# CVMI-Lab/DODA

Measured on AMD Instinct MI355X. Metric: active-voxels/sec fwd+bwd SparseConv U-Net, ScanNet 2cm, higher is better.
Workload: dtype bf16; 1 GPU; cfgs/scannet SparseConv U-Net training step (voxel pooling + fwd + CE + bwd + SGD), 2 cm voxels, 4 scenes/GPU x ~150000 active voxels, random-init weights; global_batch=4, voxels_per_gpu=601279, points_per_gpu=781042, parallelism=dp1, n_classes=20, grad_sync=deferred multi-layer wgrad + bucketed all-reduce, collectives=none (single process), prefetch_gate=off, grad_exchange=no process group

## Files before the change

doda_amd/csrc/spconv_tile.hip:

```cpp
#include "common.hpp"
#include "tilebook.hpp"
#include "spconv_common.hpp"

#ifdef DODA_TILE_STAMPS
__device__ unsigned long long doda_tile_stamp_buf[768 * 8 * 8];
extern "C" int doda_debug_tile_stamps(void *host_out, size_t bytes) {
    return (int)hipMemcpyFromSymbol(host_out, HIP_SYMBOL(doda_tile_stamp_buf), bytes);
}
#define TILE_STAMP(k)                                                                                      \
    do {                                                                                                   \
        if (tid0 == 0 && stamp_it < 8) doda_tile_stamp_buf[(blockIdx.x * 8 + stamp_it) * 8 + (k)] = wall_clock64(); \
    } while (0)
#else
#define TILE_STAMP(k) do { } while (0)
#endif

namespace {

template <bool OUT32> struct EpiPre { u32x4 res[4], bnx[4]; };
template <> struct EpiPre<false> { u32x2 res[4], bnx[4]; };

template <int S, bool OUT32, bool STATS, bool ALWAYS = false>
__device__ __forceinline__ void epi_prefetch(EpiPre<OUT32> &pre, int row0, int i, int g, int nb0, int nc, int n_out,
                                             unsigned y_bytes, const void *__restrict__ res, const EpiArgs &ep) {
    constexpr unsigned OSZ = OUT32 ? 4u : 2u;
    const unsigned col = (unsigned)(nb0 * 16 + 4 * g);
    const unsigned rl = ep.res_ld ? ep.res_ld : (unsigned)nc, bl = ep.bnx_ld ? ep.bnx_ld : (unsigned)nc;
    const unsigned dense_bytes = (unsigned)n_out * (unsigned)nc * OSZ;
    const unsigned r_bytes = ep.res_ld ? ((unsigned)(n_out - 1) * rl + (unsigned)nc) * OSZ : (ep.y_ld ? dense_bytes : y_bytes);
    const unsigned b_bytes = ep.bnx_ld ? ((unsigned)(n_out - 1) * bl + (unsigned)nc) * OSZ : (ep.y_ld ? dense_bytes : y_bytes);
    const __amdgpu_buffer_rsrc_t rs_r = __builtin_amdgcn_make_buffer_rsrc((void *)res, 0, r_bytes, 0x00020000);
    const __amdgpu_buffer_rsrc_t rs_b = __builtin_amdgcn_make_buffer_rsrc((void *)ep.bn_x, 0, b_bytes, 0x00020000);
#pragma unroll
    for (int s = 0; s < S; ++s) {
        const unsigned t = (unsigned)(row0 + s * 16 + i);
        const bool in_range = t < (unsigned)n_out && col < (unsigned)nc;
        const unsigned voff = in_range ? (t * rl + col) * OSZ : OOB;
        const unsigned voff_b = in_range ? (t * bl + col) * OSZ : OOB;
        if constexpr (ALWAYS) {
            const unsigned vr = res ? voff : OOB, vb = ep.bn_x ? voff_b : OOB;
            if constexpr (OUT32) pre.res[s] = __builtin_amdgcn_raw_buffer_load_b128(rs_r, vr, 0, 0);
            else pre.res[s] = __builtin_amdgcn_raw_buffer_load_b64(rs_r, vr, 0, 0);
            if constexpr (STATS) {
                if constexpr (OUT32) pre.bnx[s] = __builtin_amdgcn_raw_buffer_load_b128(rs_b, vb, 0, 0);
                else pre.bnx[s] = __builtin_amdgcn_raw_buffer_load_b64(rs_b, vb, 0, 0);
            }
            continue;
        }
        if (res) {
            if constexpr (OUT32) pre.res[s] = __builtin_amdgcn_raw_buffer_load_b128(rs_r, voff, 0, 0);
            else pre.res[s] = __builtin_amdgcn_raw_buffer_load_b64(rs_r, voff, 0, 0);
        }
        if (STATS && ep.bn_x) {
            if constexpr (OUT32) pre.bnx[s] = __builtin_amdgcn_raw_buffer_load_b128(rs_b, voff_b, 0, 0);
            else pre.bnx[s] = __builtin_amdgcn_raw_buffer_load_b64(rs_b, voff_b, 0, 0);
        }
    }
}

__device__ __forceinline__ f32x4 epi_unpack(const u32x4 &v) { return __builtin_bit_cast(f32x4, v); }
__device__ __forceinline__ f32x4 epi_unpack(const u32x2 &v) {
    return (f32x4){__uint_as_float(v[0] << 16), __uint_as_float(v[0] & 0xffff0000u),
                   __uint_as_float(v[1] << 16), __uint_as_float(v[1] & 0xffff0000u)};
}

template <int S, bool OUT32, bool STATS, bool BNLDS = false, int B = 0, int NBA = 1>
__device__ __forceinline__ void tile_epilogue(f32x4 (&acc)[S][NBA], const EpiPre<OUT32> &pre, int row0, int i, int g,
                                              int nb0, int nc, int n_out, __amdgpu_buffer_rsrc_t rs_y,
                                              const void *__restrict__ res, const EpiArgs &ep, f32x4 (&lst)[2],
                                              const f32x4 (*bnv_lds)[4] = nullptr) {
    constexpr unsigned OSZ = OUT32 ? 4u : 2u;
    const unsigned col = (unsigned)(nb0 * 16 + 4 * g);
    f32x4 st1 = {0.f, 0.f, 0.f, 0.f}, st2 = {0.f, 0.f, 0.f, 0.f};
    f32x4 mu = {0.f, 0.f, 0.f, 0.f}, is = mu, ga = mu, be = mu;
    if constexpr (STATS) {
        if (BNLDS && ep.bn_x) {
            mu = bnv_lds[0][g];
            is = bnv_lds[1][g];
            ga = bnv_lds[2][g];
            be = bnv_lds[3][g];
        } else if (!BNLDS && ep.bn_x) {
            const unsigned cc = col < (unsigned)nc ? col : 0u;
            mu = *reinterpret_cast<const f32x4 *>(ep.bn_mean + cc);
            is = *reinterpret_cast<const f32x4 *>(ep.bn_invstd + cc);
            if (ep.bn_relu) {
                ga = *reinterpret_cast<const f32x4 *>(ep.bn_gamma + cc);
                be = *reinterpret_cast<const f32x4 *>(ep.bn_beta + cc);
            }
        }
    }
    const unsigned yl = ep.y_ld ? ep.y_ld : (unsigned)nc;
#pragma unroll
    for (int s = 0; s < S; ++s) {
        const unsigned t = (unsigned)(row0 + s * 16 + i);
        const unsigned voff = (t < (unsigned)n_out && col < (unsigned)nc) ? (t * yl + col) * OSZ : OOB;
        f32x4 a = acc[s][B];
        if (res) a += epi_unpack(pre.res[s]);
        u32x2 packed_out = {0u, 0u};
        if constexpr (!OUT32) {
            packed_out[0] = (unsigned)f2bf(a[0]) | ((unsigned)f2bf(a[1]) << 16);
            packed_out[1] = (unsigned)f2bf(a[2]) | ((unsigned)f2bf(a[3]) << 16);
        }
        if constexpr (STATS) {
            f32x4 v = a;
            if constexpr (!OUT32) v = epi_unpack(packed_out);
            if (ep.bn_x) {
                const f32x4 xr = epi_unpack(pre.bnx[s]);
                const f32x4 xh = (xr - mu) * is;
                if (ep.bn_relu) {
                    const f32x4 yv = xh * ga + be;
#pragma unroll
                    for (int q = 0; q < 4; ++q) v[q] = yv[q] > 0.f ? v[q] : 0.f;
                }
                st1 += v;
                st2 += v * xh;
            } else {
                st1 += v;
                st2 += v * v;
            }
        }
        if constexpr (OUT32)
            __builtin_amdgcn_raw_buffer_store_b128(__builtin_bit_cast(u32x4, a), rs_y, voff, 0, 0);
        else
            __builtin_amdgcn_raw_buffer_store_b64(packed_out, rs_y, voff, 0, 0);
    }
    if constexpr (STATS) {
        lst[0] += st1;
        lst[1] += st2;
    }
}

__device__ __forceinline__ void stats_flush(f32x4 (&lst)[2], int i, int g, int wid, int nb0, int nc, const EpiArgs &ep, long long part) {
    __shared__ f32x4 sred[4][2][4];
    f32x4 st1 = lst[0], st2 = lst[1];
#pragma unroll
    for (int q = 0; q < 4; ++q) { st1[q] = row_sum16(st1[q]); st2[q] = row_sum16(st2[q]); }
    if (i == 15) { sred[wid][0][g] = st1; sred[wid][1][g] = st2; }
    doda_sync();
    const int col = nb0 * 16 + 4 * g;
    if (wid == 0 && i == 15 && col < nc) {
        const f32x4 a1 = (sred[0][0][g] + sred[1][0][g]) + (sred[2][0][g] + sred[3][0][g]);
        const f32x4 a2 = (sred[0][1][g] + sred[1][1][g]) + (sred[2][1][g] + sred[3][1][g]);
        stats_emit(ep, part, nc, col, a1, a2);
    }
    doda_sync();
}

template <int MODE, bool OUT32, bool STATS, int MAXNB, bool DUAL = false>
__global__ __launch_bounds__(256, MODE == 0 ? 3 : 2) void conv_tile(const void *__restrict__ x, unsigned x_bytes,
                                                 const void *__restrict__ wp, unsigned wp_bytes, int nc, int NB,
                                                 const int32_t *__restrict__ tbl, int ld, int n_out,
                                                 const TileBookView tb, void *__restrict__ y, unsigned y_bytes,
                                                 const void *__restrict__ res, const EpiArgs ep) {
    constexpr bool WIDE = MODE != 0;
    static_assert(MODE != 2 || OUT32, "fp32 features have fp32 outputs");
    static_assert(!DUAL || (MODE == 1 && (MAXNB == 2 || MAXNB == 4 || !STATS)), "two channel blocks per pass: bf16, 64-byte rows");
    static_assert(MAXNB != 4 || DUAL, "statistics of four channel blocks: two dual passes");
    constexpr int NBA = DUAL ? 2 : 1;
    constexpr int S = 4, NU = WIDE ? TB_K : (TB_K + 1) / 2;
    constexpr int RB = WIDE ? 64 : 32;
    constexpr int PPR = RB / 16;
    constexpr int CAP = WIDE ? TB_CAP64 : TB_LMAX;
    constexpr int NLJ = PPR;
    constexpr int NRL = 4 * NLJ;
    constexpr int NLP = TB_LIDX_BYTES / 16;
    constexpr int NLI = (NLP + 255) / 256;
    __shared__ __attribute__((aligned(16))) unsigned char rows_s[(CAP + 1) * RB];
    __shared__ __attribute__((aligned(16))) unsigned lidx_s[TB_T * TB_LW];
    static_assert(MAXNB == 1 || MAXNB == 2 || MAXNB == 4, "statistics of one, two or (dual passes) four channel blocks");
    f32x4 lst[STATS ? MAXNB : 1][2];
#pragma unroll
    for (int b = 0; b < (STATS ? MAXNB : 1); ++b) lst[b][0] = lst[b][1] = (f32x4){0.f, 0.f, 0.f, 0.f};

    const int tid0 = threadIdx.x, wid = __builtin_amdgcn_readfirstlane(tid0 >> 6);
    const __amdgpu_buffer_rsrc_t rs_x = __builtin_amdgcn_make_buffer_rsrc((void *)x, 0, x_bytes, 0x00020000);
    const __amdgpu_buffer_rsrc_t rs_w = __builtin_amdgcn_make_buffer_rsrc((void *)wp, 0, wp_bytes, 0x00020000);
    const __amdgpu_buffer_rsrc_t rs_y = __builtin_amdgcn_make_buffer_rsrc((void *)y, 0, y_bytes, 0x00020000);
    const __amdgpu_buffer_rsrc_t rs_t = __builtin_amdgcn_make_buffer_rsrc((void *)tbl, 0, (unsigned)TB_K * (unsigned)ld * 4u, 0x00020000);

    const int L = gridDim.x >> 3, xcd = blockIdx.x & 7, slot = blockIdx.x >> 3;
    const int qn = tb.nt >> 3, rn = tb.nt & 7;
    const int lo = xcd < rn ? xcd * (qn + 1) : rn * (qn + 1) + (xcd - rn) * qn;
    const int cnt = qn + (xcd < rn ? 1 : 0);

    auto entry_of = [&](int j, int k, int tid) { return j * (256 / PPR) + tid / PPR + 256 * k; };
    auto load_list = [&](int tile, int tid, unsigned (&rid)[NRL]) {
        const u32x4 *ul4 = reinterpret_cast<const u32x4 *>(tb.ulist + (size_t)tile * TB_UMAX);
#pragma unroll
        for (int j = 0; j < NLJ; ++j) {
            const u32x4 v = ul4[j * (256 / PPR) + tid / PPR];
#pragma unroll
            for (int k = 0; k < 4; ++k) rid[4 * j + k] = v[k];
        }
    };
    unsigned rid[NRL];
    int U = 0;
    if (slot < cnt) {
        load_list(lo + slot, tid0, rid);
        U = tb.ucount[lo + slot];
    }
#ifdef DODA_TILE_STAMPS
    int stamp_it = -1;
#endif
    for (int tt = slot; tt < cnt; tt += L) {
        const int tile = lo + tt, t0 = tile * TB_T;
#ifdef DODA_TILE_STAMPS
        ++stamp_it;
#endif
        TILE_STAMP(0);
        int tid = tid0;
        asm volatile("" : "+v"(tid));
        const int lane = tid & 63, i = lane & 15, g = lane >> 4;
        const bool staged = U <= CAP;
        const int row0 = t0 + wid * 64;
        const unsigned half = (unsigned)(WIDE ? g : (g & 1)) * 16u;
        unsigned lane_w = WIDE ? (unsigned)lane * 16u
                               : (unsigned)(g >> 1) * (unsigned)NB * 512u + (unsigned)((g & 1) * 16 + i) * 16u;
        auto loadw = [&](int u, int b = 0) {
            return __builtin_amdgcn_raw_buffer_load_b128(rs_w, (unsigned)u * (unsigned)NB * 1024u + lane_w + (unsigned)b * (WIDE ? 1024u : 512u), 0, 0);
        };
        EpiPre<OUT32> pre;
        epi_prefetch<S, OUT32, STATS>(pre, row0, i, g, 0, nc, n_out, y_bytes, res, ep);

        if (staged) {
            u32x4 rr[NRL];
#pragma unroll
            for (int k = 0; k < NRL; ++k)
                rr[k] = __builtin_amdgcn_raw_buffer_load_b128(rs_x, rid[k] * (unsigned)RB + (unsigned)(tid & (PPR - 1)) * 16u, 0, 0);
            u32x4 li4[NLI];
            const u32x4 *li = reinterpret_cast<const u32x4 *>(tb.lidx + (size_t)tile * (TB_T * TB_LW));
#pragma unroll
            for (int k = 0; k < NLI; ++k) {
                const int e = k * 256 + tid;
                li4[k] = li[e < NLP ? e : 0];
            }
            if (tt + L < cnt) {
                load_list(tile + L, tid, rid);
                U = tb.ucount[tile + L];
            }
#pragma unroll
            for (int k = 0; k < NLI; ++k) {
                const int e = k * 256 + tid;
                if (e < NLP) reinterpret_cast<u32x4 *>(lidx_s)[e] = li4[k];
            }
            if (tid < PPR) reinterpret_cast<u32x4 *>(rows_s)[tid] = (u32x4){0u, 0u, 0u, 0u};
#pragma unroll
            for (int k = 0; k < NRL; ++k) {
                const int e = entry_of(k >> 2, k & 3, tid);
                if (e < CAP) reinterpret_cast<u32x4 *>(rows_s)[PPR + e * PPR + (tid & (PPR - 1))] = rr[k];
            }
        } else {
            static_assert((CAP + 1) * RB >= TB_K * TB_T * 4, "the table slice fits the row buffer");
            int te[TB_K];
            unsigned ldv = (unsigned)ld;
            asm volatile("" : "+s"(ldv));
#pragma unroll
            for (int o = 0; o < TB_K; ++o) {
                const unsigned voff = (unsigned)(t0 + tid) < (unsigned)n_out ? ((unsigned)o * ldv + (unsigned)(t0 + tid)) * 4u : OOB;
                te[o] = (int)__builtin_amdgcn_raw_buffer_load_b32(rs_t, voff, 0, 0);
            }
            if (tt + L < cnt) {
                load_list(tile + L, tid, rid);
                U = tb.ucount[tile + L];
            }
            int *tab_s = reinterpret_cast<int *>(rows_s);
#pragma unroll
            for (int o = 0; o < TB_K; ++o) tab_s[o * TB_T + tid] = (unsigned)(t0 + tid) < (unsigned)n_out ? te[o] : -1;
        }
        TILE_STAMP(1);
        doda_sync();
        TILE_STAMP(2);

        for (int nb0 = 0; nb0 < NB; nb0 += NBA) {
            if (nb0 > 0) {
                lane_w += (WIDE ? 1024u : 512u) * (unsigned)NBA;
                epi_prefetch<S, OUT32, STATS>(pre, row0, i, g, nb0, nc, n_out, y_bytes, res, ep);
            }

            f32x4 acc[S][NBA];
#pragma unroll
            for (int s = 0; s < S; ++s)
#pragma unroll
                for (int b = 0; b < NBA; ++b) acc[s][b] = (f32x4){0.f, 0.f, 0.f, 0.f};
            if (staged) {
                const unsigned *my = lidx_s + wid * 64 + tb_lsigma(i) * 4 + ((!WIDE && (g >> 1)) ? 5 * TB_T : 0);
                auto loadp = [&](int plane) { return *reinterpret_cast<const u32x4 *>(my + plane * TB_T); };
                constexpr int NSTR = WIDE ? 2 : 1;
                u32x4 lw[NSTR][2];
                auto word_of = [&](int u) -> const u32x4 & { return WIDE ? lw[u & 1][((u >> 1) / 3) & 1] : lw[0][(u / 3) & 1]; };
                auto fetch = [&](int u, u32x4 (&xa)[S]) {
                    const unsigned sh = WIDE ? 10u * (unsigned)((u >> 1) % 3) : 10u * (unsigned)(u % 3);
                    const u32x4 &l = word_of(u);
#pragma unroll
                    for (int s = 0; s < S; ++s)
                        xa[s] = *reinterpret_cast<const u32x4 *>(rows_s + ((__builtin_amdgcn_ubfe(l[s], sh, 10u) * (unsigned)RB) | half));
                };
                auto next_word = [&](int u) {
                    if constexpr (WIDE) {
                        const int p = u & 1, k = (u >> 1) / 3;
                        if ((u >> 1) % 3 == 0 && 2 * (3 * (k + 1)) + p < TB_K) lw[p][(k + 1) & 1] = loadp(5 * p + k + 1);
                    } else {
                        const int k = u / 3;
                        if (u % 3 == 0 && 3 * (k + 1) < NU) lw[0][(k + 1) & 1] = loadp(k + 1);
                    }
                };
                u32x4 xa[2][S], wr[4][NBA];
#pragma unroll
                for (int u = 0; u < 3; ++u)
#pragma unroll
                    for (int b = 0; b < NBA; ++b) wr[u][b] = loadw(u, b);
                lw[0][0] = loadp(0);
                if constexpr (WIDE) lw[1][0] = loadp(5);
                fetch(0, xa[0]);
#pragma unroll
                for (int u = 0; u < NU; ++u) {
                    if (u + 1 < NU) fetch(u + 1, xa[(u + 1) & 1]);
                    next_word(u);
                    if (u + 3 < NU) {
#pragma unroll
                        for (int b = 0; b < NBA; ++b) wr[(u + 3) & 3][b] = loadw(u + 3, b);
                    }
                    __builtin_amdgcn_sched_barrier(0);
#pragma unroll
                    for (int s = 0; s < S; ++s) {
#pragma unroll
                        for (int b = 0; b < NBA; ++b) {
                            if constexpr (MODE == 2) mma_f32_k16<false>(acc[s][b], wr[u & 3][b], xa[u & 1][s]);
                            else mma_bf16_k32(acc[s][b], wr[u & 3][b], xa[u & 1][s]);
                        }
                    }
                    __builtin_amdgcn_sched_barrier(0);
                }
            } else {
                const int *tab_s = reinterpret_cast<const int *>(rows_s) + wid * 64 + i;
                auto ldi = [&](int u, int (&d)[S]) {
                    const int osel = WIDE ? u : 2 * u + (g >> 1);
#pragma unroll
                    for (int s = 0; s < S; ++s) d[s] = osel < TB_K ? tab_s[osel * TB_T + s * 16] : -1;
                };
                auto ldx = [&](const int (&d)[S], u32x4 (&xr)[S]) {
#pragma unroll
                    for (int s = 0; s < S; ++s)
                        xr[s] = __builtin_amdgcn_raw_buffer_load_b128(rs_x, d[s] >= 0 ? (unsigned)d[s] * (unsigned)RB + half : OOB, 0, 0);
                };
                int ix[3][S];
                u32x4 xo[2][S];
                ldi(0, ix[0]);
                ldi(1, ix[1]);
                ldx(ix[0], xo[0]);
#pragma unroll
                for (int u = 0; u < NU; ++u) {
                    if (u + 2 < NU) ldi(u + 2, ix[(u + 2) % 3]);
                    if (u + 1 < NU) ldx(ix[(u + 1) % 3], xo[(u + 1) & 1]);
                    u32x4 wu[NBA];
#pragma unroll
                    for (int b = 0; b < NBA; ++b) wu[b] = loadw(u, b);
#pragma unroll
                    for (int s = 0; s < S; ++s) {
#pragma unroll
                        for (int b = 0; b < NBA; ++b) {
                            if constexpr (MODE == 2) mma_f32_k16<false>(acc[s][b], wu[b], xo[u & 1][s]);
                            else mma_bf16_k32(acc[s][b], wu[b], xo[u & 1][s]);
                        }
                    }
                }
            }
            TILE_STAMP(3);
            if constexpr (DUAL) {
                EpiPre<OUT32> pre1;
                epi_prefetch<S, OUT32, STATS>(pre1, row0, i, g, nb0 + 1, nc, n_out, y_bytes, res, ep);
                if (MAXNB == 4 && nb0 == 2) {
                    tile_epilogue<S, OUT32, STATS, false, 0, NBA>(acc, pre, row0, i, g, nb0, nc, n_out, rs_y, res, ep, lst[STATS && MAXNB == 4 ? 2 : 0]);
                    tile_epilogue<S, OUT32, STATS, false, 1, NBA>(acc, pre1, row0, i, g, nb0 + 1, nc, n_out, rs_y, res, ep, lst[STATS && MAXNB == 4 ? 3 : 0]);
                } else {
                    tile_epilogue<S, OUT32, STATS, false, 0, NBA>(acc, pre, row0, i, g, nb0, nc, n_out, rs_y, res, ep, lst[0]);
                    tile_epilogue<S, OUT32, STATS, false, 1, NBA>(acc, pre1, row0, i, g, nb0 + 1, nc, n_out, rs_y, res, ep, lst[STATS && MAXNB > 1 ? 1 : 0]);
                }
            } else {
                if (nb0 == 0) tile_epilogue<S, OUT32, STATS>(acc, pre, row0, i, g, nb0, nc, n_out, rs_y, res, ep, lst[0]);
                else tile_epilogue<S, OUT32, STATS>(acc, pre, row0, i, g, nb0, nc, n_out, rs_y, res, ep, lst[STATS ? MAXNB - 1 : 0]);
            }
        }
        TILE_STAMP(4);
        doda_sync();
        TILE_STAMP(5);
    }
    if constexpr (STATS) {
        const int lane = tid0 & 63, i = lane & 15, g = lane >> 4;
        stats_flush(lst[0], i, g, wid, 0, nc, ep, (long long)blockIdx.x);
#pragma unroll
        for (int b = 1; b < MAXNB; ++b)
            if (b < NB) stats_flush(lst[b], i, g, wid, b, nc, ep, (long long)blockIdx.x);
    }
}

template <bool OUT32, bool STATS>
__global__ __launch_bounds__(256, 2) void conv_tile16(const void *__restrict__ x, unsigned x_bytes,
                                                      const void *__restrict__ wp, unsigned wp_bytes, int nc,
                                                      const int32_t *__restrict__ tbl, int ld, int n_out,
                                                      const TileBookView tb, void *__restrict__ y, unsigned y_bytes,
                                                      const void *__restrict__ res, const EpiArgs ep) {
    constexpr int S = 4, NU = (TB_K + 1) / 2, RB = 32, PPR = 2, CAP = TB_LMAX, NLJ = PPR, NRL = 4 * NLJ;
    constexpr int NLP = TB_LIDX_BYTES / 16, NLI = (NLP + 255) / 256;
    __shared__ __attribute__((aligned(16))) unsigned char rows_s[(CAP + 1) * RB];
    __shared__ __attribute__((aligned(16))) unsigned lidx_s[TB_T * TB_LW];
    __shared__ f32x4 bnv_s[4][4];
    f32x4 lst[2] = {{0.f, 0.f, 0.f, 0.f}, {0.f, 0.f, 0.f, 0.f}};

    const int tid = threadIdx.x, wid = __builtin_amdgcn_readfirstlane(tid >> 6);
    if constexpr (STATS) {
        if (ep.bn_x && tid < 64) {
            const int v = tid >> 4, c = tid & 15;
            const float *src = v == 0 ? ep.bn_mean : v == 1 ? ep.bn_invstd : v == 2 ? ep.bn_gamma : ep.bn_beta;
            reinterpret_cast<float *>(bnv_s)[v * 16 + c] = (src && c < nc) ? src[c] : 0.f;
        }
    }
    const int lane = tid & 63, i = lane & 15, g = lane >> 4;
    const __amdgpu_buffer_rsrc_t rs_x = __builtin_amdgcn_make_buffer_rsrc((void *)x, 0, x_bytes, 0x00020000);
    const __amdgpu_buffer_rsrc_t rs_w = __builtin_amdgcn_make_buffer_rsrc((void *)wp, 0, wp_bytes, 0x00020000);
    const __amdgpu_buffer_rsrc_t rs_y = __builtin_amdgcn_make_buffer_rsrc((void *)y, 0, y_bytes, 0x00020000);
    const __amdgpu_buffer_rsrc_t rs_t = __builtin_amdgcn_make_buffer_rsrc((void *)tbl, 0, (unsigned)TB_K * (unsigned)ld * 4u, 0x00020000);

    const int L = gridDim.x >> 3, xcd = blockIdx.x & 7, slot = blockIdx.x >> 3;
    const int qn = tb.nt >> 3, rn = tb.nt & 7;
    const int lo = xcd < rn ? xcd * (qn + 1) : rn * (qn + 1) + (xcd - rn) * qn;
    const int cnt = qn + (xcd < rn ? 1 : 0);
    const unsigned half = (unsigned)(g & 1) * 16u;

    u32x4 wr[NU];
    {
        const unsigned lane_w = (unsigned)(g >> 1) * 512u + (unsigned)((g & 1) * 16 + i) * 16u;
#pragma unroll
        for (int u = 0; u < NU; ++u) wr[u] = __builtin_amdgcn_raw_buffer_load_b128(rs_w, (unsigned)u * 1024u + lane_w, 0, 0);
    }

    const __amdgpu_buffer_rsrc_t rs_ul = __builtin_amdgcn_make_buffer_rsrc((void *)tb.ulist, 0, (unsigned)tb.nt * (unsigned)(TB_UMAX * 4), 0x00020000);
    const __amdgpu_buffer_rsrc_t rs_li = __builtin_amdgcn_make_buffer_rsrc((void *)tb.lidx, 0, (unsigned)tb.nt * (unsigned)TB_LIDX_BYTES, 0x00020000);
    auto entry_of = [&](int j, int k) { return j * (256 / PPR) + tid / PPR + 256 * k; };
    const __amdgpu_buffer_rsrc_t rs_uc = __builtin_amdgcn_make_buffer_rsrc((void *)tb.ucount, 0, (unsigned)tb.nt * 4u, 0x00020000);
    auto load_list = [&](int tile, unsigned (&rid)[NRL]) {
        const unsigned base = tile >= 0 ? (unsigned)tile * (unsigned)(TB_UMAX * 4) : OOB;
#pragma unroll
        for (int j = 0; j < NLJ; ++j) {
            const u32x4 v = __builtin_amdgcn_raw_buffer_load_b128(rs_ul, base + (unsigned)(j * (256 / PPR) + tid / PPR) * 16u, 0, 0);
#pragma unroll
            for (int k = 0; k < 4; ++k) rid[4 * j + k] = v[k];
        }
    };
    auto request = [&](int tile, unsigned none, const unsigned (&rid)[NRL], u32x4 (&rr)[NRL], u32x4 (&li4)[NLI], unsigned &count) {
        count = __builtin_amdgcn_raw_buffer_load_b32(rs_uc, none ? OOB : (unsigned)tile * 4u, 0, 0);
#pragma unroll
        for (int k = 0; k < NRL; ++k) {
            const unsigned r = rid[k] | none;
            rr[k] = __builtin_amdgcn_raw_buffer_load_b128(rs_x, r < 0x04000000u ? r * (unsigned)RB + (unsigned)(tid & (PPR - 1)) * 16u : OOB, 0, 0);
        }
        const unsigned base = none ? OOB : (unsigned)tile * (unsigned)TB_LIDX_BYTES;
#pragma unroll
        for (int k = 0; k < NLI; ++k) {
            const int e = k * 256 + tid;
            li4[k] = __builtin_amdgcn_raw_buffer_load_b128(rs_li, base + (unsigned)(e < NLP ? e : 0) * 16u, 0, 0);
        }
    };

    unsigned rid[NRL];
    u32x4 rr[NRL], li4[NLI];
    unsigned U = 0;
    load_list(slot < cnt ? lo + slot : -1, rid);
    asm volatile("" : "+v"(wr[0]), "+v"(wr[1]), "+v"(wr[2]), "+v"(wr[3]), "+v"(wr[4]), "+v"(wr[5]), "+v"(wr[6]), "+v"(wr[7]),
                      "+v"(wr[8]), "+v"(wr[9]), "+v"(wr[10]), "+v"(wr[11]), "+v"(wr[12]), "+v"(wr[13]),
                      "+v"(rid[0]), "+v"(rid[1]), "+v"(rid[2]), "+v"(rid[3]), "+v"(rid[4]), "+v"(rid[5]), "+v"(rid[6]), "+v"(rid[7]));
    static_assert(NU == 14 && NRL == 8, "operand list of the asm above");
    if (slot >= cnt) return;
    request(lo + slot, 0u, rid, rr, li4, U);
    load_list(slot + L < cnt ? lo + slot + L : -1, rid);
    __builtin_amdgcn_sched_barrier(0);
#pragma unroll
    for (int k = 0; k < S; ++k) __builtin_amdgcn_raw_buffer_store_b32((unsigned)k, rs_y, OOB + 16u * (unsigned)k, 0, 0);
    __builtin_amdgcn_sched_barrier(0);
#ifdef DODA_TILE_STAMPS
    const int tid0 = tid;
    int stamp_it = -1;
#endif
    for (int tt = slot; tt < cnt; tt += L) {
        const int tile = lo + tt, t0 = tile * TB_T;
#ifdef DODA_TILE_STAMPS
        ++stamp_it;
#endif
        TILE_STAMP(0);
        const bool staged = __builtin_amdgcn_readfirstlane(U) <= (unsigned)CAP;
        const int row0 = t0 + wid * 64;
        if (staged) {
#pragma unroll
            for (int k = 0; k < NLI; ++k) {
                const int e = k * 256 + tid;
                if (e < NLP) reinterpret_cast<u32x4 *>(lidx_s)[e] = li4[k];
            }
            if (tid < PPR) reinterpret_cast<u32x4 *>(rows_s)[tid] = (u32x4){0u, 0u, 0u, 0u};
#pragma unroll
            for (int k = 0; k < NRL; ++k) {
                const int e = entry_of(k >> 2, k & 3);
                if (e < CAP) reinterpret_cast<u32x4 *>(rows_s)[PPR + e * PPR + (tid & (PPR - 1))] = rr[k];
            }
        } else {
            static_assert((CAP + 1) * RB >= TB_K * TB_T * 4, "the table slice fits the row buffer");
            int te[TB_K];
#pragma unroll
            for (int o = 0; o < TB_K; ++o) {
                const unsigned voff = (unsigned)(t0 + tid) < (unsigned)n_out ? ((unsigned)o * (unsigned)ld + (unsigned)(t0 + tid)) * 4u : OOB;
                te[o] = (int)__builtin_amdgcn_raw_buffer_load_b32(rs_t, voff, 0, 0);
            }
            int *tab_s = reinterpret_cast<int *>(rows_s);
#pragma unroll
            for (int o = 0; o < TB_K; ++o) tab_s[o * TB_T + tid] = (unsigned)(t0 + tid) < (unsigned)n_out ? te[o] : -1;
        }
        TILE_STAMP(1);
        doda_sync();
        TILE_STAMP(2);

        EpiPre<OUT32> pre;
        epi_prefetch<S, OUT32, STATS, true>(pre, row0, i, g, 0, nc, n_out, y_bytes, res, ep);
        unsigned Unext;
        request(tile + L, tt + L < cnt ? 0u : 0xffffffffu, rid, rr, li4, Unext);
        load_list(tt + 2 * L < cnt ? tile + 2 * L : -1, rid);

        f32x4 acc[S][1];
#pragma unroll
        for (int s = 0; s < S; ++s) acc[s][0] = (f32x4){0.f, 0.f, 0.f, 0.f};
        if (staged) {
            const unsigned *my = lidx_s + wid * 64 + tb_lsigma(i) * 4 + ((g >> 1) ? 5 * TB_T : 0);
            auto loadp = [&](int k) { return *reinterpret_cast<const u32x4 *>(my + k * TB_T); };
            u32x4 lw[2];
            auto fetch = [&](int u, u32x4 (&xa)[S]) {
                const u32x4 &l = lw[(u / 3) & 1];
#pragma unroll
                for (int s = 0; s < S; ++s)
                    xa[s] = *reinterpret_cast<const u32x4 *>(rows_s + ((__builtin_amdgcn_ubfe(l[s], 10u * (unsigned)(u % 3), 10u) * (unsigned)RB) | half));
            };
            u32x4 xa[2][S];
            lw[0] = loadp(0);
            fetch(0, xa[0]);
#pragma unroll
            for (int u = 0; u < NU; ++u) {
                if (u + 1 < NU) fetch(u + 1, xa[(u + 1) & 1]);
                if (u % 3 == 0 && 3 * (u / 3 + 1) < NU) lw[(u / 3 + 1) & 1] = loadp(u / 3 + 1);
                __builtin_amdgcn_sched_barrier(0);
#pragma unroll
                for (int s = 0; s < S; ++s) mma_bf16_k32(acc[s][0], wr[u], xa[u & 1][s]);
                __builtin_amdgcn_sched_barrier(0);
            }
        } else {
            const int *tab_s = reinterpret_cast<const int *>(rows_s) + wid * 64 + i;
            auto ldi = [&](int u, int (&d)[S]) {
                const int osel = 2 * u + (g >> 1);
#pragma unroll
                for (int s = 0; s < S; ++s) d[s] = osel < TB_K ? tab_s[osel * TB_T + s * 16] : -1;
            };
            auto ldx = [&](const int (&d)[S], u32x4 (&xr)[S]) {
#pragma unroll
                for (int s = 0; s < S; ++s)
                    xr[s] = __builtin_amdgcn_raw_buffer_load_b128(rs_x, d[s] >= 0 ? (unsigned)d[s] * (unsigned)RB + half : OOB, 0, 0);
            };
            int ix[3][S];
            u32x4 xo[2][S];
            ldi(0, ix[0]);
            ldi(1, ix[1]);
            ldx(ix[0], xo[0]);
#pragma unroll
            for (int u = 0; u < NU; ++u) {
                if (u + 2 < NU) ldi(u + 2, ix[(u + 2) % 3]);
                if (u + 1 < NU) ldx(ix[(u + 1) % 3], xo[(u + 1) & 1]);
#pragma unroll
                for (int s = 0; s < S; ++s) mma_bf16_k32(acc[s][0], wr[u], xo[u & 1][s]);
            }
        }
        TILE_STAMP(3);
        tile_epilogue<S, OUT32, STATS, true>(acc, pre, row0, i, g, 0, nc, n_out, rs_y, res, ep, lst, bnv_s);
        U = Unext;
        TILE_STAMP(4);
        doda_sync();
        TILE_STAMP(5);
    }
    if constexpr (STATS) stats_flush(lst, i, g, wid, 0, nc, ep, (long long)blockIdx.x);
}

template <bool OUT32, bool STATS>
__global__ __launch_bounds__(256) void conv_up32(const void *__restrict__ x, unsigned x_bytes, const void *__restrict__ wp,
                                                 unsigned wp_bytes, int nc, int NB, int K, const int32_t *__restrict__ tbl, int ld,
                                                 int n_out, void *__restrict__ y, unsigned y_bytes, const void *__restrict__ res,
                                                 const EpiArgs ep) {
    constexpr int S = 4, KMAX = 8;
    const int tid = threadIdx.x, wid = __builtin_amdgcn_readfirstlane(tid >> 6);
    const int lane = tid & 63, i = lane & 15, g = lane >> 4;
    const __amdgpu_buffer_rsrc_t rs_x = __builtin_amdgcn_make_buffer_rsrc((void *)x, 0, x_bytes, 0x00020000);
    const __amdgpu_buffer_rsrc_t rs_w = __builtin_amdgcn_make_buffer_rsrc((void *)wp, 0, wp_bytes, 0x00020000);
    const __amdgpu_buffer_rsrc_t rs_y = __builtin_amdgcn_make_buffer_rsrc((void *)y, 0, y_bytes, 0x00020000);
    const __amdgpu_buffer_rsrc_t rs_t = __builtin_amdgcn_make_buffer_rsrc((void *)tbl, 0, (unsigned)K * (unsigned)ld * 4u, 0x00020000);
    const int row0 = (int)blockIdx.x * TB_T + wid * 64;
    int te[KMAX];
    {
        const unsigned r = (unsigned)(row0 + lane);
#pragma unroll
        for (int o = 0; o < KMAX; ++o) {
            const bool ok = o < K && r < (unsigned)n_out;
            const int v = (int)__builtin_amdgcn_raw_buffer_load_b32(rs_t, ok ? ((unsigned)o * (unsigned)ld + r) * 4u : OOB, 0, 0);
            te[o] = ok ? v : -1;
        }
    }
    for (int nb0 = 0; nb0 < NB; ++nb0) {
        EpiPre<OUT32> pre;
        epi_prefetch<S, OUT32, STATS>(pre, row0, i, g, nb0, nc, n_out, y_bytes, res, ep);
        u32x4 wr[KMAX];
#pragma unroll
        for (int o = 0; o < KMAX; ++o)
            wr[o] = __builtin_amdgcn_raw_buffer_load_b128(rs_w, o < K ? ((unsigned)(o * NB + nb0) * 64u + (unsigned)lane) * 16u : OOB, 0, 0);
        f32x4 acc[S][1];
#pragma unroll
        for (int s = 0; s < S; ++s) acc[s][0] = (f32x4){0.f, 0.f, 0.f, 0.f};
        for (int j = 0; j < KMAX; ++j) {
            int code = -1, seen = 0;
#pragma unroll
            for (int o = 0; o < KMAX; ++o) {
                const bool v = te[o] >= 0;
                code = (v && seen == j) ? ((te[o] << 3) | o) : code;
                seen += v ? 1 : 0;
            }
            if (__builtin_amdgcn_ballot_w64(code >= 0) == 0ull) break;
            int cs[S];
            u32x4 xr[S];
#pragma unroll
            for (int s = 0; s < S; ++s) {
                cs[s] = __builtin_amdgcn_ds_bpermute((s * 16 + i) * 4, code);
                xr[s] = __builtin_amdgcn_raw_buffer_load_b128(rs_x, cs[s] >= 0 ? (unsigned)(cs[s] >> 3) * 64u + (unsigned)g * 16u : OOB, 0, 0);
            }
#pragma unroll
            for (int o = 0; o < KMAX; ++o) {
                if (__builtin_amdgcn_ballot_w64(code >= 0 && (code & 7) == o) == 0ull) continue;
#pragma unroll
                for (int s = 0; s < S; ++s) {
                    const bool mine = cs[s] >= 0 && (cs[s] & 7) == o;
                    u32x4 b;
#pragma unroll
                    for (int q = 0; q < 4; ++q) b[q] = mine ? xr[s][q] : 0u;
                    mma_bf16_k32(acc[s][0], wr[o], b);
                }
            }
        }
        f32x4 lst[2] = {{0.f, 0.f, 0.f, 0.f}, {0.f, 0.f, 0.f, 0.f}};
        tile_epilogue<S, OUT32, STATS>(acc, pre, row0, i, g, nb0, nc, n_out, rs_y, res, ep, lst);
        if constexpr (STATS) stats_flush(lst, i, g, wid, nb0, nc, ep, (long long)blockIdx.x);
    }
}

constexpr int BT_MAX_GROUPS = 768;
bool g_dual = !(getenv("DODA_TILE_DUAL") && getenv("DODA_TILE_DUAL")[0] == '0');
bool g_pipeline = true;
bool g_up = !(getenv("DODA_CONV_UP") && getenv("DODA_CONV_UP")[0] == '0');
bool dual_blocks() { return g_dual; }
constexpr int T16_MAX_GROUPS = 512;
int tile16_min_tiles() {
    static const int v = [] {
        const char *e = getenv("DODA_TILE16_MIN_TILES");
        const int m = e && *e ? atoi(e) : BT_MAX_GROUPS + 1;
        return m < T16_MAX_GROUPS ? T16_MAX_GROUPS : m;
    }();
    return v;
}

bool g_use_tile = true;

}

bool doda_tile::enabled() { return g_use_tile; }
void doda_tile::set_enabled(bool on) { g_use_tile = on; }
bool doda_tile::pipeline_enabled() { return g_pipeline; }
void doda_tile::set_pipeline(bool on) { g_pipeline = on; }
bool doda_tile::dual_enabled() { return g_dual; }
void doda_tile::set_dual(bool on) { g_dual = on; }
bool doda_tile::up_enabled() { return g_up; }
void doda_tile::set_up(bool on) { g_up = on; }

int doda_tile::launch_conv_up32(bool out32, const void *x, unsigned xb, const void *wp, unsigned wpb, int nc, int NB, int K,
                                const int32_t *tbl, int ld, int n_out, void *y, unsigned yb, const void *res, const EpiArgs &ep,
                                int *n_part, hipStream_t s) {
    const int groups = (n_out + TB_T - 1) / TB_T;
    if (n_part) *n_part = groups;
    const dim3 grid(groups), block(256);
#define GU(O32, ST) hipLaunchKernelGGL((conv_up32<O32, ST>), grid, block, 0, s, x, xb, wp, wpb, nc, NB, K, tbl, ld, n_out, y, yb, res, ep)
    if (out32) { if (ep.stats) GU(true, true); else GU(true, false); }
    else { if (ep.stats) GU(false, true); else GU(false, false); }
#undef GU
    return doda_check_launch();
}

int doda_tile::launch_conv_tile(int mode, bool out32, const void *x, unsigned xb, const void *wp, unsigned wpb, int nc, int NB,
                                const int32_t *tbl, int ld, int n_out, const void *tilebook, void *y, unsigned yb,
                                const void *res, const EpiArgs &ep_in, int *n_part, hipStream_t s) {
    const TileBookView tb = tilebook_view(const_cast<void *>(tilebook), n_out);
    if (mode == 0 && NB == 1 && g_pipeline && tb.nt >= tile16_min_tiles()) {
        const int groups16 = T16_MAX_GROUPS;
        if (n_part) *n_part = groups16;
        const dim3 grid(groups16), block(256);
        const EpiArgs &ep = ep_in;
#define G16(O32, ST)                                                                               \
    hipLaunchKernelGGL((conv_tile16<O32, ST>), grid, block, 0, s, x, xb, wp, wpb, nc, tbl, ld, n_out, tb, y, yb, res, ep)
        if (out32) { if (ep.stats) G16(true, true); else G16(true, false); }
        else { if (ep.stats) G16(false, true); else G16(false, false); }
#undef G16
        return doda_check_launch();
    }
    int groups = (tb.nt + 7) / 8 * 8;
    const int max_groups = mode == 0 ? BT_MAX_GROUPS : BT_MAX_GROUPS * 2 / 3;
    if (groups > max_groups) groups = max_groups;
    const dim3 grid(groups), block(256);
    if (ep_in.stats && NB > 2 && !(mode == 1 && NB == 4 && dual_blocks())) return DODA_ERR_UNSUPPORTED;
    const bool two = NB > 1 && ep_in.stats;
    if (n_part) *n_part = groups;
    const EpiArgs &ep = ep_in;
#define GT1(M, O32, ST, NBS)                                                                       \
    hipLaunchKernelGGL((conv_tile<M, O32, ST, NBS>), grid, block, 0, s, x, xb, wp, wpb, nc, NB, tbl, ld, n_out, tb, y, yb, res, ep)
#define GTD(O32, ST)                                                                               \
    hipLaunchKernelGGL((conv_tile<1, O32, ST, 2, true>), grid, block, 0, s, x, xb, wp, wpb, nc, NB, tbl, ld, n_out, tb, y, yb, res, ep)
#define GT(M, O32, ST)                                                                             \
    do {                                                                                           \
        if (ST && two) GT1(M, O32, ST, 2); else GT1(M, O32, ST, 1);                                \
    } while (0)
#define GM(M)                                                                                      \
    do {                                                                                           \
        if (out32) { if (ep.stats) GT(M, true, true); else GT(M, true, false); }                   \
        else { if (ep.stats) GT(M, false, true); else GT(M, false, false); }                       \
    } while (0)
    if (mode == 2) { if (ep.stats) GT(2, true, true); else GT(2, true, false); }
    else if (mode == 1 && NB == 2 && dual_blocks()) {
        if (out32) { if (ep.stats) GTD(true, true); else GTD(true, false); }
        else { if (ep.stats) GTD(false, true); else GTD(false, false); }
    }
    else if (mode == 1 && NB == 4 && dual_blocks()) {
#define GTQ(O32, ST) hipLaunchKernelGGL((conv_tile<1, O32, ST, 4, true>), grid, block, 0, s, x, xb, wp, wpb, nc, NB, tbl, ld, n_out, tb, y, yb, res, ep)
        if (out32) { if (ep.stats) GTQ(true, true); else GTD(true, false); }
        else { if (ep.stats) GTQ(false, true); else GTD(false, false); }
#undef GTQ
    }
    else if (mode == 1) GM(1);
    else GM(0);
#undef GM
#undef GT
#undef GT1
#undef GTD
    return doda_check_launch();
}
```

Baseline: 136.6 million voxels/s.

## Add conv_tile32 kernel with cross-tile prefetch for 64-byte-row tile convolutions

Adds a new persistent tile convolution kernel for mode 1 (64-byte bf16 rows) with one or two channel blocks. It prefetches the next tile's row list, gathered rows and local indices while the current tile computes, and software-pipelines LDS row fetches and weight loads around the MFMA loop. It also handles two channel blocks in one pass (dual) and sets occupancy hints via launch bounds. The new path is on by default for mode 1 with NB 1, or NB 2 when dual blocks are enabled. In exchange it holds more live registers for the prefetched state, which may lower occupancy.

New measurement: 137.8 million voxels/s (median of 6 runs). Within noise of the previous version (+0.9%).

```diff
diff --git a/doda_amd/csrc/spconv_tile.hip b/doda_amd/csrc/spconv_tile.hip
--- a/doda_amd/csrc/spconv_tile.hip
+++ b/doda_amd/csrc/spconv_tile.hip
@@ -583,6 +583,242 @@
     if constexpr (STATS) stats_flush(lst, i, g, wid, 0, nc, ep, (long long)blockIdx.x);
 }
 
+template <int MODE, bool OUT32, bool STATS, int NBT, bool DUAL>
+__global__ __launch_bounds__(256, MODE == 0 ? 3 : 2) void conv_tile32(const void *__restrict__ x, unsigned x_bytes,
+                                                                   const void *__restrict__ wp, unsigned wp_bytes, int nc,
+                                                                   const int32_t *__restrict__ tbl, int ld, int n_out,
+                                                                   const TileBookView tb, void *__restrict__ y, unsigned y_bytes,
+                                                                   const void *__restrict__ res, const EpiArgs ep) {
+    constexpr bool WIDE = MODE != 0;
+    static_assert(MODE == 0 || MODE == 1, "bf16 rows (MODE 2 keeps conv_tile)");
+    static_assert(!DUAL || MODE == 1, "two channel blocks per pass: 64-byte rows");
+    constexpr int NBA = DUAL ? 2 : 1, NP = NBT / NBA;
+    static_assert(NP * NBA == NBT && NP <= 2, "one or two passes");
+    constexpr int S = 4, NU = WIDE ? TB_K : (TB_K + 1) / 2, RB = WIDE ? 64 : 32, PPR = RB / 16;
+    constexpr int CAP = WIDE ? TB_CAP64 : TB_LMAX, NLJ = PPR, NRL = 4 * NLJ;
+    constexpr int NLP = TB_LIDX_BYTES / 16, NLI = (NLP + 255) / 256;
+    constexpr unsigned WB = WIDE ? 1024u : 512u;
+    __shared__ __attribute__((aligned(16))) unsigned char rows_s[(CAP + 1) * RB];
+    __shared__ __attribute__((aligned(16))) unsigned lidx_s[TB_T * TB_LW];
+    __shared__ f32x4 bnv_s[STATS ? NBT * 4 : 1][4];
+    f32x4 lst[STATS ? NBT : 1][2];
+#pragma unroll
+    for (int b = 0; b < (STATS ? NBT : 1); ++b) lst[b][0] = lst[b][1] = (f32x4){0.f, 0.f, 0.f, 0.f};
+
+    const int tid0 = threadIdx.x, wid = __builtin_amdgcn_readfirstlane(tid0 >> 6);
+    if constexpr (STATS) {
+        if (ep.bn_x && tid0 < 64 * NBT) {
+            const int v = (tid0 >> 4) & 3, c = (tid0 >> 6) * 16 + (tid0 & 15);
+            const float *src = v == 0 ? ep.bn_mean : v == 1 ? ep.bn_invstd : v == 2 ? ep.bn_gamma : ep.bn_beta;
+            reinterpret_cast<float *>(bnv_s)[tid0] = (src && c < nc) ? src[c] : 0.f;
+        }
+    }
+    const __amdgpu_buffer_rsrc_t rs_x = __builtin_amdgcn_make_buffer_rsrc((void *)x, 0, x_bytes, 0x00020000);
+    const __amdgpu_buffer_rsrc_t rs_w = __builtin_amdgcn_make_buffer_rsrc((void *)wp, 0, wp_bytes, 0x00020000);
+    const __amdgpu_buffer_rsrc_t rs_y = __builtin_amdgcn_make_buffer_rsrc((void *)y, 0, y_bytes, 0x00020000);
+    const __amdgpu_buffer_rsrc_t rs_t = __builtin_amdgcn_make_buffer_rsrc((void *)tbl, 0, (unsigned)TB_K * (unsigned)ld * 4u, 0x00020000);
+    const __amdgpu_buffer_rsrc_t rs_ul = __builtin_amdgcn_make_buffer_rsrc((void *)tb.ulist, 0, (unsigned)tb.nt * (unsigned)(TB_UMAX * 4), 0x00020000);
+    const __amdgpu_buffer_rsrc_t rs_li = __builtin_amdgcn_make_buffer_rsrc((void *)tb.lidx, 0, (unsigned)tb.nt * (unsigned)TB_LIDX_BYTES, 0x00020000);
+    const __amdgpu_buffer_rsrc_t rs_uc = __builtin_amdgcn_make_buffer_rsrc((void *)tb.ucount, 0, (unsigned)tb.nt * 4u, 0x00020000);
+
+    const int L = gridDim.x >> 3, xcd = blockIdx.x & 7, slot = blockIdx.x >> 3;
+    const int qn = tb.nt >> 3, rn = tb.nt & 7;
+    const int lo = xcd < rn ? xcd * (qn + 1) : rn * (qn + 1) + (xcd - rn) * qn;
+    const int cnt = qn + (xcd < rn ? 1 : 0);
+
+    auto entry_of = [&](int j, int k, int tid) { return j * (256 / PPR) + tid / PPR + 256 * k; };
+    auto load_list = [&](int tile, int tid, unsigned (&rid)[NRL]) {
+        const unsigned base = tile >= 0 ? (unsigned)tile * (unsigned)(TB_UMAX * 4) : OOB;
+#pragma unroll
+        for (int j = 0; j < NLJ; ++j) {
+            const u32x4 v = __builtin_amdgcn_raw_buffer_load_b128(rs_ul, base + (unsigned)(j * (256 / PPR) + tid / PPR) * 16u, 0, 0);
+#pragma unroll
+            for (int k = 0; k < 4; ++k) rid[4 * j + k] = v[k];
+        }
+    };
+    auto request = [&](int tile, unsigned none, int tid, const unsigned (&rid)[NRL], u32x4 (&rr)[NRL], u32x4 (&li4)[NLI],
+                       unsigned &count) {
+        count = __builtin_amdgcn_raw_buffer_load_b32(rs_uc, none ? OOB : (unsigned)tile * 4u, 0, 0);
+#pragma unroll
+        for (int k = 0; k < NRL; ++k) {
+            const unsigned r = rid[k] | none;
+            rr[k] = __builtin_amdgcn_raw_buffer_load_b128(rs_x, r < 0x04000000u ? r * (unsigned)RB + (unsigned)(tid & (PPR - 1)) * 16u : OOB, 0, 0);
+        }
+        const unsigned base = none ? OOB : (unsigned)tile * (unsigned)TB_LIDX_BYTES;
+#pragma unroll
+        for (int k = 0; k < NLI; ++k) {
+            const int e = k * 256 + tid;
+            li4[k] = __builtin_amdgcn_raw_buffer_load_b128(rs_li, base + (unsigned)(e < NLP ? e : 0) * 16u, 0, 0);
+        }
+    };
+
+    unsigned rid[NRL];
+    u32x4 rr[NRL], li4[NLI];
+    unsigned U = 0;
+    load_list(slot < cnt ? lo + slot : -1, tid0, rid);
+    request(lo + slot, slot < cnt ? 0u : 0xffffffffu, tid0, rid, rr, li4, U);
+    load_list(slot + L < cnt ? lo + slot + L : -1, tid0, rid);
+    __builtin_amdgcn_sched_barrier(0);
+#pragma unroll
+    for (int k = 0; k < S * NBT; ++k) __builtin_amdgcn_raw_buffer_store_b32((unsigned)k, rs_y, OOB + 16u * (unsigned)k, 0, 0);
+    __builtin_amdgcn_sched_barrier(0);
+#ifdef DODA_TILE_STAMPS
+    int stamp_it = -1;
+#endif
+    for (int tt = slot; tt < cnt; tt += L) {
+        const int tile = lo + tt, t0 = tile * TB_T;
+#ifdef DODA_TILE_STAMPS
+        ++stamp_it;
+#endif
+        TILE_STAMP(0);
+        int tid = tid0;
+        asm volatile("" : "+v"(tid));
+        const int lane = tid & 63, i = lane & 15, g = lane >> 4;
+        const bool staged = __builtin_amdgcn_readfirstlane(U) <= (unsigned)CAP;
+        const int row0 = t0 + wid * 64;
+        const unsigned half = (unsigned)(WIDE ? g : (g & 1)) * 16u;
+        const unsigned lane_w = WIDE ? (unsigned)lane * 16u : (unsigned)(g >> 1) * (unsigned)NBT * 512u + (unsigned)((g & 1) * 16 + i) * 16u;
+        auto loadw = [&](int u, int b) {
+            return __builtin_amdgcn_raw_buffer_load_b128(rs_w, (unsigned)u * (unsigned)NBT * 1024u + lane_w + (unsigned)b * WB, 0, 0);
+        };
+        if (staged) {
+#pragma unroll
+            for (int k = 0; k < NLI; ++k) {
+                const int e = k * 256 + tid;
+                if (e < NLP) reinterpret_cast<u32x4 *>(lidx_s)[e] = li4[k];
+            }
+            if (tid < PPR) reinterpret_cast<u32x4 *>(rows_s)[tid] = (u32x4){0u, 0u, 0u, 0u};
+#pragma unroll
+            for (int k = 0; k < NRL; ++k) {
+                const int e = entry_of(k >> 2, k & 3, tid);
+                if (e < CAP) reinterpret_cast<u32x4 *>(rows_s)[PPR + e * PPR + (tid & (PPR - 1))] = rr[k];
+            }
+        } else {
+            static_assert((CAP + 1) * RB >= TB_K * TB_T * 4, "the table slice fits the row buffer");
+            int te[TB_K];
+#pragma unroll
+            for (int o = 0; o < TB_K; ++o) {
+                const unsigned voff = (unsigned)(t0 + tid) < (unsigned)n_out ? ((unsigned)o * (unsigned)ld + (unsigned)(t0 + tid)) * 4u : OOB;
+                te[o] = (int)__builtin_amdgcn_raw_buffer_load_b32(rs_t, voff, 0, 0);
+            }
+            int *tab_s = reinterpret_cast<int *>(rows_s);
+#pragma unroll
+            for (int o = 0; o < TB_K; ++o) tab_s[o * TB_T + tid] = (unsigned)(t0 + tid) < (unsigned)n_out ? te[o] : -1;
+        }
+        TILE_STAMP(1);
+        doda_sync();
+        TILE_STAMP(2);
+
+        unsigned Unext = 0;
+#pragma unroll
+        for (int p = 0; p < NP; ++p) {
+            const int nb0 = p * NBA;
+            EpiPre<OUT32> pre[NBA];
+#pragma unroll
+            for (int b = 0; b < NBA; ++b) epi_prefetch<S, OUT32, STATS, true>(pre[b], row0, i, g, nb0 + b, nc, n_out, y_bytes, res, ep);
+            f32x4 acc[S][NBA];
+#pragma unroll
+            for (int s = 0; s < S; ++s)
+#pragma unroll
+                for (int b = 0; b < NBA; ++b) acc[s][b] = (f32x4){0.f, 0.f, 0.f, 0.f};
+            if (staged) {
+                const unsigned *my = lidx_s + wid * 64 + tb_lsigma(i) * 4 + ((!WIDE && (g >> 1)) ? 5 * TB_T : 0);
+                auto loadp = [&](int plane) { return *reinterpret_cast<const u32x4 *>(my + plane * TB_T); };
+                constexpr int NSTR = WIDE ? 2 : 1;
+                u32x4 lw[NSTR][2];
+                auto word_of = [&](int u) -> const u32x4 & { return WIDE ? lw[u & 1][((u >> 1) / 3) & 1] : lw[0][(u / 3) & 1]; };
+                auto fetch = [&](int u, u32x4 (&xa)[S]) {
+                    const unsigned sh = WIDE ? 10u * (unsigned)((u >> 1) % 3) : 10u * (unsigned)(u % 3);
+                    const u32x4 &l = word_of(u);
+#pragma unroll
+                    for (int s = 0; s < S; ++s)
+                        xa[s] = *reinterpret_cast<const u32x4 *>(rows_s + ((__builtin_amdgcn_ubfe(l[s], sh, 10u) * (unsigned)RB) | half));
+                };
+                auto next_word = [&](int u) {
+                    if constexpr (WIDE) {
+                        const int q = u & 1, k = (u >> 1) / 3;
+                        if ((u >> 1) % 3 == 0 && 2 * (3 * (k + 1)) + q < TB_K) lw[q][(k + 1) & 1] = loadp(5 * q + k + 1);
+                    } else {
+                        const int k = u / 3;
+                        if (u % 3 == 0 && 3 * (k + 1) < NU) lw[0][(k + 1) & 1] = loadp(k + 1);
+                    }
+                };
+                u32x4 xa[2][S], wr[4][NBA];
+#pragma unroll
+                for (int u = 0; u < 3; ++u)
+#pragma unroll
+                    for (int b = 0; b < NBA; ++b) wr[u][b] = loadw(u, nb0 + b);
+                lw[0][0] = loadp(0);
+                if constexpr (WIDE) lw[1][0] = loadp(5);
+                fetch(0, xa[0]);
+#pragma unroll
+                for (int u = 0; u < NU; ++u) {
+                    if (u + 1 < NU) fetch(u + 1, xa[(u + 1) & 1]);
+                    next_word(u);
+                    if (u + 3 < NU) {
+#pragma unroll
+                        for (int b = 0; b < NBA; ++b) wr[(u + 3) & 3][b] = loadw(u + 3, nb0 + b);
+                    }
+                    __builtin_amdgcn_sched_barrier(0);
+#pragma unroll
+                    for (int s = 0; s < S; ++s)
+#pragma unroll
+                        for (int b = 0; b < NBA; ++b) mma_bf16_k32(acc[s][b], wr[u & 3][b], xa[u & 1][s]);
+                    __builtin_amdgcn_sched_barrier(0);
+                }
+            } else {
+                const int *tab_s = reinterpret_cast<const int *>(rows_s) + wid * 64 + i;
+                auto ldi = [&](int u, int (&d)[S]) {
+                    const int osel = WIDE ? u : 2 * u + (g >> 1);
+#pragma unroll
+                    for (int s = 0; s < S; ++s) d[s] = osel < TB_K ? tab_s[osel * TB_T + s * 16] : -1;
+                };
+                auto ldx = [&](const int (&d)[S], u32x4 (&xr)[S]) {
+#pragma unroll
+                    for (int s = 0; s < S; ++s)
+                        xr[s] = __builtin_amdgcn_raw_buffer_load_b128(rs_x, d[s] >= 0 ? (unsigned)d[s] * (unsigned)RB + half : OOB, 0, 0);
+                };
+                int ix[3][S];
+                u32x4 xo[2][S];
+                ldi(0, ix[0]);
+                ldi(1, ix[1]);
+                ldx(ix[0], xo[0]);
+#pragma unroll
+                for (int u = 0; u < NU; ++u) {
+                    if (u + 2 < NU) ldi(u + 2, ix[(u + 2) % 3]);
+                    if (u + 1 < NU) ldx(ix[(u + 1) % 3], xo[(u + 1) & 1]);
+                    u32x4 wu[NBA];
+#pragma unroll
+                    for (int b = 0; b < NBA; ++b) wu[b] = loadw(u, nb0 + b);
+#pragma unroll
+                    for (int s = 0; s < S; ++s)
+#pragma unroll
+                        for (int b = 0; b < NBA; ++b) mma_bf16_k32(acc[s][b], wu[b], xo[u & 1][s]);
+                }
+            }
+            if (p == NP - 1) {
+                request(tile + L, tt + L < cnt ? 0u : 0xffffffffu, tid, rid, rr, li4, Unext);
+                load_list(tt + 2 * L < cnt ? tile + 2 * L : -1, tid, rid);
+            }
+            TILE_STAMP(3);
+            tile_epilogue<S, OUT32, STATS, true, 0, NBA>(acc, pre[0], row0, i, g, nb0, nc, n_out, rs_y, res, ep, lst[STATS ? nb0 : 0],
+                                                          bnv_s + (STATS ? nb0 * 4 : 0));
+            if constexpr (DUAL)
+                tile_epilogue<S, OUT32, STATS, true, 1, NBA>(acc, pre[1], row0, i, g, nb0 + 1, nc, n_out, rs_y, res, ep,
+                                                              lst[STATS ? nb0 + 1 : 0], bnv_s + (STATS ? (nb0 + 1) * 4 : 0));
+        }
+        U = Unext;
+        TILE_STAMP(4);
+        doda_sync();
+        TILE_STAMP(5);
+    }
+    if constexpr (STATS) {
+        const int lane = tid0 & 63, i = lane & 15, g = lane >> 4;
+#pragma unroll
+        for (int b = 0; b < NBT; ++b) stats_flush(lst[b], i, g, wid, b, nc, ep, (long long)blockIdx.x);
+    }
+}
+
 template <bool OUT32, bool STATS>
 __global__ __launch_bounds__(256) void conv_up32(const void *__restrict__ x, unsigned x_bytes, const void *__restrict__ wp,
                                                  unsigned wp_bytes, int nc, int NB, int K, const int32_t *__restrict__ tbl, int ld,
@@ -667,6 +903,14 @@
 }
 
 bool g_use_tile = true;
+bool g_tile32 = !(getenv("DODA_TILE32") && getenv("DODA_TILE32")[0] == '0');
+int tile32_min_tiles() {
+    static const int v = [] {
+        const char *e = getenv("DODA_TILE32_MIN_TILES");
+        return e && *e ? atoi(e) : 0;
+    }();
+    return v;
+}
 
 }
 
@@ -712,6 +956,24 @@
     const int max_groups = mode == 0 ? BT_MAX_GROUPS : BT_MAX_GROUPS * 2 / 3;
     if (groups > max_groups) groups = max_groups;
     const dim3 grid(groups), block(256);
+    const bool t32 = g_pipeline && g_tile32 && tb.nt >= tile32_min_tiles() && tb.nt > 0 &&
+                     mode == 1 && (NB == 1 || (NB == 2 && dual_blocks()));
+    if (t32) {
+        if (n_part) *n_part = groups;
+        const EpiArgs &ep = ep_in;
+#define G32(M, O32, ST, NBT, DU)                                                                   \
+    hipLaunchKernelGGL((conv_tile32<M, O32, ST, NBT, DU>), grid, block, 0, s, x, xb, wp, wpb, nc, tbl, ld, n_out, tb, y, yb, res, ep)
+#define G32S(M, NBT, DU)                                                                           \
+    do {                                                                                           \
+        if (out32) { if (ep.stats) G32(M, true, true, NBT, DU); else G32(M, true, false, NBT, DU); } \
+        else { if (ep.stats) G32(M, false, true, NBT, DU); else G32(M, false, false, NBT, DU); }  \
+    } while (0)
+        if (NB == 1) G32S(1, 1, false);
+        else G32S(1, 2, true);
+#undef G32S
+#undef G32
+        return doda_check_launch();
+    }
     if (ep_in.stats && NB > 2 && !(mode == 1 && NB == 4 && dual_blocks())) return DODA_ERR_UNSUPPORTED;
     const bool two = NB > 1 && ep_in.stats;
     if (n_part) *n_part = groups;
```
